# WangWen-Believer/DR-SLAM

Hardware: AMD Instinct MI355X
Metric: RGB-D frames/sec (extract+match) at 640x480 (higher is better)
Workload: dtype u8

## Files before the change

### dr_slam_amd/csrc/drfe_internal.h

```cpp
#ifndef DRFE_INTERNAL_H
#define DRFE_INTERNAL_H

#include <hip/hip_runtime.h>
#ifndef DRFE_NO_ROCTX
#include <roctracer/roctx.h>
#else
static inline int roctxRangePushA(const char*) { return 0; }
static inline int roctxRangePop() { return 0; }
#endif
#include <stdint.h>
#include <time.h>
#include <string>
#include <vector>

#include "../../include/drfe.h"
#include "../../include/drfe_debug.h"

#define DRFE_MAX_LEVELS 16
#define DRFE_EDGE 19
#define DRFE_HALF_PATCH 15
#define DRFE_GRID_COLS 64
#define DRFE_GRID_ROWS 48
#define DRFE_GRID_CELLS (DRFE_GRID_COLS * DRFE_GRID_ROWS)
#define DRFE_FASTC_MAX_EW 38
#define DRFE_FASTC_MAX_RPL 12
#define DRFE_FAST_MAX_WIN 60
#define DRFE_QT_MAX_NODES 1024
#define DRFE_MATCH_MAX_CAND 256

struct DevLevel {
    int w, h;
    int pyrPitch, pyrOff;
    int blurPitch, blurOff;
    int quota;
    int minBX, minBY, maxBX, maxBY;
    int nCols, nRows, wCell, hCell;
    int candCap, candOff;
    int kpCap, kpOff;
    int nIni;
    float hX;
    float scale;
    float kpSize;
    int xtabOff, ytabOff;
    int xwinOff, ywinOff;
    int resizeLds;
    int cellBegin, cellEnd;
    int tileBegin, tileEnd;
};

struct DevGeom {
    int nlevels;
    int iniTh, minTh;
    int imgW, imgH;
    int pyrSlotBytes, blurSlotBytes;
    int candSlotElems, kpSlotElems;
    int totalCells, totalTiles;
    int fastMaxWh;
    int fastCols;
    int fastColsSmall;
    int fastColsRows;
    DevLevel lv[DRFE_MAX_LEVELS];
};

#ifndef DRFE_CC_LINE
#define DRFE_CC_LINE 32
#endif
#define DRFE_CC_SLOT (DRFE_MAX_LEVELS * DRFE_CC_LINE)
#define DRFE_CC_IDX(slot, level) ((size_t)(slot) * DRFE_CC_SLOT + (size_t)(level) * DRFE_CC_LINE)

struct FastCell {
    uint16_t x0, y0;
    uint8_t ww, wh;
    uint8_t level, off;
    uint16_t offX, offY;
    uint32_t cellIdx;
    uint32_t srcOff;
    uint32_t pitch;
    uint32_t candOff, candCap;
    uint8_t ncp, nrb, rpl, pad;
    uint32_t ncpMagic;
};

struct BlurTile { uint16_t tx, ty; uint16_t level, pad; };

struct ResizeTap { uint16_t s0, s1; int16_t w0, w1; };

#include "undistort_math.h"

struct drfe_ctx {
    drfe_config cfg;
    int device;
    hipStream_t stream;
    std::string err;

    std::vector<float> scale, invScale, sigma2, invSigma2;
    std::vector<int> quota;
    int umax[DRFE_HALF_PATCH + 1];
    DevGeom geom;
// ... 128 lines not shown
{
    (void)roctxRangePushA(drfe_stage_name(stage));
    if (c->profile) { (void)hipEventRecord(c->ev[stage][0], s); c->evUsed[stage] = true; }
}
static inline void prof_end(drfe_ctx* c, int stage, hipStream_t s)
{
    if (c->profile) (void)hipEventRecord(c->ev[stage][1], s);
    (void)roctxRangePop();
}
struct DrfeRange {
    explicit DrfeRange(const char* name) { (void)roctxRangePushA(name); }
    ~DrfeRange() { (void)roctxRangePop(); }
};

static inline hipError_t drfe_event_wait_sleeping(hipEvent_t ev)
{
    for (int spins = 0;; spins++) {
        const hipError_t e = hipEventQuery(ev);
        if (e != hipErrorNotReady) return e;
        if (spins < 4) continue;
        struct timespec ts = {0, spins < 40 ? 20000 : 100000};
        nanosleep(&ts, nullptr);
    }
}

void drfe_pool_cpu_add(int pool, long long ns);
struct DrfePoolCpuScope {
    int pool; struct timespec t0;
    explicit DrfePoolCpuScope(int p) : pool(p) { clock_gettime(CLOCK_THREAD_CPUTIME_ID, &t0); }
    ~DrfePoolCpuScope() { struct timespec t1; clock_gettime(CLOCK_THREAD_CPUTIME_ID, &t1); drfe_pool_cpu_add(pool, (t1.tv_sec - t0.tv_sec) * 1000000000LL + (t1.tv_nsec - t0.tv_nsec)); }
};

hipError_t drfe_long_kernel_stream(hipStream_t* s, int part);

int drfe_default_host_threads();
void drfe_cape_lanes_free(drfe_ctx* c);
void drfe_bow_slot_invalidate(drfe_ctx* c, int slot);
void drfe_one_shot_free(drfe_ctx* c);
void drfe_frame_lanes_free(drfe_ctx* c);

int drfe_build_tables(drfe_ctx* c);
int drfe_build_geometry(drfe_ctx* c, int w, int h, DevGeom* g, std::vector<FastCell>* cells,
                        std::vector<BlurTile>* tiles, std::vector<ResizeTap>* taps);

hipError_t drfe_launch_orb(drfe_ctx* c, const uint8_t* d_gray, size_t frameStride, size_t rowStride, int nframes,
                           hipStream_t s);
hipError_t drfe_launch_glue(drfe_ctx* c, const uint16_t* d_depth, size_t frameStride, size_t rowStride,
                            const drfe_camera& cam, int nframes, hipStream_t s);
hipError_t drfe_launch_grid(drfe_ctx* c, const drfe_camera& cam, int nframes, hipStream_t s);
hipError_t drfe_launch_kp_pixels(drfe_ctx* c, int nframes, uint32_t* d_uv, hipStream_t s);
hipError_t drfe_launch_match_consecutive(drfe_ctx* c, const drfe_camera& cam, float th, int mono, int checkOri,
                                         int nframes, hipStream_t s);

#define DRFE_RESIZE_LDS_WD 88
#define DRFE_RESIZE_LDS_ROWS 24
static inline uint32_t drfe_div_magic(uint32_t d) { return d <= 1 ? 0u : (uint32_t)(((1ull << 32) + d - 1) / d); }
#if defined(__HIPCC__)
__device__ __forceinline__ uint32_t drfe_div_by(uint32_t n, uint32_t d, uint32_t magic)
{
    if (!magic) return n;
    uint32_t q = __umulhi(n, magic);
    if (q * d > n) q--;
    return q;
}
__device__ __forceinline__ int drfe_wave_incl_scan(int v, int lane)
{
    v += __builtin_amdgcn_update_dpp(0, v, 0x111, 0xf, 0xf, true);
    v += __builtin_amdgcn_update_dpp(0, v, 0x112, 0xf, 0xf, true);
    v += __builtin_amdgcn_update_dpp(0, v, 0x114, 0xf, 0xf, true);
    v += __builtin_amdgcn_update_dpp(0, v, 0x118, 0xf, 0xf, true);
    const int t0 = __builtin_amdgcn_readlane(v, 15), t1 = __builtin_amdgcn_readlane(v, 31), t2 = __builtin_amdgcn_readlane(v, 47);
    return v + (lane >= 16 ? t0 : 0) + (lane >= 32 ? t1 : 0) + (lane >= 48 ? t2 : 0);
}

__device__ __forceinline__ int drfe_wave_sum_i32(int v)
{
    v += __builtin_amdgcn_update_dpp(0, v, 0xB1, 0xf, 0xf, false);
    v += __builtin_amdgcn_update_dpp(0, v, 0x4E, 0xf, 0xf, false);
    v += __builtin_amdgcn_update_dpp(0, v, 0x124, 0xf, 0xf, false);
    v += __builtin_amdgcn_update_dpp(0, v, 0x128, 0xf, 0xf, false);
    return __builtin_amdgcn_readlane(v, 0) + __builtin_amdgcn_readlane(v, 16) + __builtin_amdgcn_readlane(v, 32) + __builtin_amdgcn_readlane(v, 48);
}
__device__ __forceinline__ uint32_t drfe_wave_min_u32(uint32_t v)
{
    v = min(v, (uint32_t)__builtin_amdgcn_update_dpp(0, (int)v, 0xB1, 0xf, 0xf, false));
    v = min(v, (uint32_t)__builtin_amdgcn_update_dpp(0, (int)v, 0x4E, 0xf, 0xf, false));
    v = min(v, (uint32_t)__builtin_amdgcn_update_dpp(0, (int)v, 0x124, 0xf, 0xf, false));
    v = min(v, (uint32_t)__builtin_amdgcn_update_dpp(0, (int)v, 0x128, 0xf, 0xf, false));
    const uint32_t a = (uint32_t)__builtin_amdgcn_readlane((int)v, 0), b = (uint32_t)__builtin_amdgcn_readlane((int)v, 16),
                   c = (uint32_t)__builtin_amdgcn_readlane((int)v, 32), d = (uint32_t)__builtin_amdgcn_readlane((int)v, 48);
    return min(min(a, b), min(c, d));
}

__device__ __forceinline__ void drfe_xcd_swizzle_2d(uint32_t magic, int& lx, int& ly)
{
    const uint32_t gx = gridDim.x, nwg = gx * gridDim.y;
    const uint32_t orig = blockIdx.y * gx + blockIdx.x;
    const uint32_t q = nwg >> 3, r = nwg & 7, xcd = orig & 7, j = orig >> 3;
    const uint32_t swz = (xcd < r ? xcd * (q + 1) : r * (q + 1) + (xcd - r) * q) + j;
    const uint32_t y = drfe_div_by(swz, gx, magic);
    lx = (int)(swz - y * gx);
    ly = (int)y;
}
__device__ __forceinline__ void drfe_xcd_swizzle_3d(uint32_t magicXY, uint32_t magicX, int& lx, int& ly, int& lz)
{
    const uint32_t gx = gridDim.x, gxy = gx * gridDim.y, nwg = gxy * gridDim.z;
    const uint32_t orig = blockIdx.z * gxy + blockIdx.y * gx + blockIdx.x;
    const uint32_t q = nwg >> 3, r = nwg & 7, xcd = orig & 7, j = orig >> 3;
// ... 29 lines not shown
```

### dr_slam_amd/csrc/orb_geometry.cpp

```cpp
#include "drfe_internal.h"
#include "../../include/drfe_math.h"

#include <algorithm>
#include <cmath>

static inline int align_up(int v, int a) { return (v + a - 1) / a * a; }

int drfe_build_tables(drfe_ctx* c)
{
    const int nl = c->cfg.nlevels;
    const double sfd = (double)c->cfg.scale_factor;
    c->scale.assign(nl, 1.f); c->sigma2.assign(nl, 1.f);
    c->invScale.assign(nl, 1.f); c->invSigma2.assign(nl, 1.f);
    for (int i = 1; i < nl; i++) {
        c->scale[i] = (float)(c->scale[i - 1] * sfd);
        c->sigma2[i] = c->scale[i] * c->scale[i];
    }
    for (int i = 0; i < nl; i++) {
        c->invScale[i] = 1.0f / c->scale[i];
        c->invSigma2[i] = 1.0f / c->sigma2[i];
    }
    c->quota.assign(nl, 0);
    const float factor = (float)(1.0f / sfd);
    float want = c->cfg.nfeatures * (1 - factor) / (1 - (float)std::pow((double)factor, (double)nl));
    int sum = 0;
    for (int l = 0; l < nl - 1; l++) {
        c->quota[l] = drfe_round_half_even(want);
        sum += c->quota[l];
        want *= factor;
    }
    c->quota[nl - 1] = std::max(c->cfg.nfeatures - sum, 0);
    const int hp = DRFE_HALF_PATCH;
    for (int v = 0; v <= hp; v++) c->umax[v] = 0;
    const int vmax = (int)std::floor(hp * std::sqrt(2.f) / 2 + 1);
    const int vmin = (int)std::ceil(hp * std::sqrt(2.f) / 2);
    const double hp2 = hp * hp;
    for (int v = 0; v <= vmax; ++v) c->umax[v] = drfe_round_half_even_d(std::sqrt(hp2 - v * v));
    for (int v = hp, v0 = 0; v >= vmin; --v) {
        while (c->umax[v0] == c->umax[v0 + 1]) ++v0;
        c->umax[v] = v0;
        ++v0;
    }
    return DRFE_OK;
}

static void build_taps_axis(int src, int dst, std::vector<ResizeTap>* out)
{
    const double inv = (double)dst / src;
    const double scale = 1. / inv;
    for (int d = 0; d < dst; d++) {
        float f = (float)((d + 0.5) * scale - 0.5);
        int s = (int)std::floor(f);
        f -= s;
        if (s < 0) { s = 0; f = 0; }
        if (s >= src - 1) { s = src - 1; f = 0; }
        ResizeTap t;
        t.s0 = (uint16_t)s;
        t.s1 = (uint16_t)std::min(s + 1, src - 1);
        int w0 = drfe_round_half_even((1.f - f) * 2048.f), w1 = drfe_round_half_even(f * 2048.f);
        t.w0 = (int16_t)std::min(32767, std::max(-32768, w0));
        t.w1 = (int16_t)std::min(32767, std::max(-32768, w1));
        out->push_back(t);
    }
}

static void build_taps(int src, int dst, int padded, std::vector<ResizeTap>* out)
{
    std::vector<ResizeTap> axis;
    build_taps_axis(src, dst, &axis);
    if (out->size() & 1) out->push_back(ResizeTap{0, 0, 0, 0});
    const int bordered = dst + 2 * DRFE_EDGE;
    for (int b = 0; b < padded; b++) {
        if (b >= bordered) { ResizeTap z = out->back(); z.w0 = z.w1 = 0; out->push_back(z); continue; }
        int p = b - DRFE_EDGE;
        if (p < 0) p = -p;
        if (p >= dst) p = 2 * (dst - 1) - p;
        out->push_back(axis[p]);
    }
}

int drfe_build_geometry(drfe_ctx* c, int w, int h, DevGeom* g, std::vector<FastCell>* cells,
                        std::vector<BlurTile>* tiles, std::vector<ResizeTap>* taps)
{
    const int nl = c->cfg.nlevels;
    g->nlevels = nl;
    g->iniTh = c->cfg.ini_th_fast;
    g->minTh = c->cfg.min_th_fast;
    g->imgW = w; g->imgH = h;
    g->fastMaxWh = 7;
    g->fastCols = 1;
    g->fastColsRows = 7;
    int pyrOff = 0, blurOff = 0, candOff = 0, kpOff = 0;
    if (cells) cells->clear();
    if (tiles) tiles->clear();
    if (taps) taps->clear();
    for (int l = 0; l < nl; l++) {
        DevLevel& L = g->lv[l];
        L.w = drfe_round_half_even((float)w * c->invScale[l]);
        L.h = drfe_round_half_even((float)h * c->invScale[l]);
        L.quota = c->quota[l];
        L.scale = c->scale[l];
        L.kpSize = (float)(int)(31 * c->scale[l]);
        L.minBX = DRFE_EDGE - 3; L.minBY = DRFE_EDGE - 3;
        L.maxBX = L.w - DRFE_EDGE + 3; L.maxBY = L.h - DRFE_EDGE + 3;
        const float width = (float)(L.maxBX - L.minBX), height = (float)(L.maxBY - L.minBY);
        L.nCols = (int)(width / 30.f);
        L.nRows = (int)(height / 30.f);
        if (L.nCols <= 0 || L.nRows <= 0) {
            c->err = "pyramid level " + std::to_string(l) + " is smaller than one 30-px FAST cell";
            return DRFE_ERR_INVALID;
        }
        L.wCell = (int)std::ceil(width / L.nCols);
        L.hCell = (int)std::ceil(height / L.nRows);
        if (L.wCell + 6 > DRFE_FAST_MAX_WIN || L.hCell + 6 > DRFE_FAST_MAX_WIN) {
            c->err = "FAST cell window exceeds the LDS tile";
            return DRFE_ERR_INVALID;
        }
        L.nIni = (int)std::round((float)(L.maxBX - L.minBX) / (L.maxBY - L.minBY));
        if (L.nIni < 1) {
            c->err = "frame aspect ratio gives zero quadtree root nodes (reference divides by zero)";
            return DRFE_ERR_INVALID;
        }
        L.hX = (float)(L.maxBX - L.minBX) / L.nIni;
        L.pyrPitch = align_up(L.w + 2 * DRFE_EDGE, 64);
        L.pyrOff = pyrOff;
        pyrOff += align_up(L.pyrPitch * (L.h + 2 * DRFE_EDGE), 256);
        L.blurPitch = (L.w + DRFE_BTILE_W - 1) / DRFE_BTILE_W;
        L.blurOff = blurOff;
        blurOff += align_up(L.blurPitch * ((L.h + DRFE_BTILE_H - 1) / DRFE_BTILE_H) * 128, 256);
        L.cellBegin = cells ? (int)cells->size() : 0;
// ... 6 lines not shown
            for (int j = 0; j < L.nCols; j++) {
                const float iniX = (float)(L.minBX + j * L.wCell);
                float maxX = iniX + L.wCell + 6;
                if (iniX >= L.maxBX - 6) continue;
                if (maxX > L.maxBX) maxX = (float)L.maxBX;
                FastCell fc;
                fc.x0 = (uint16_t)iniX; fc.y0 = (uint16_t)iniY;
                const int ww = (int)maxX - (int)iniX, wh = (int)maxY - (int)iniY;
                if (ww < 7 || wh < 7) continue;
                fc.ww = (uint8_t)ww; fc.wh = (uint8_t)wh;
                fc.level = (uint8_t)l;
                fc.off = (uint8_t)((fc.x0 + DRFE_EDGE) & 3);
                fc.srcOff = (uint32_t)(L.pyrOff + (fc.y0 + DRFE_EDGE) * L.pyrPitch + (fc.x0 + DRFE_EDGE - fc.off));
                fc.pitch = (uint32_t)L.pyrPitch;
                fc.candOff = 0; fc.candCap = 0;
                fc.offX = (uint16_t)(j * L.wCell); fc.offY = (uint16_t)(i * L.hCell);
                fc.cellIdx = (uint32_t)(i * L.nCols + j);
                {
                    const int ew = ww - 6, eh = wh - 6;
                    const int ncp = (ew + 1) / 2, nrb0 = std::min(64 / ncp, eh);
                    const int rpl = (eh + nrb0 - 1) / nrb0;
                    const int nrb = (eh + rpl - 1) / rpl;
                    fc.ncp = (uint8_t)ncp; fc.nrb = (uint8_t)nrb; fc.rpl = (uint8_t)rpl; fc.pad = 0;
                    fc.ncpMagic = (uint32_t)((65536 + ncp - 1) / ncp);
                    g->fastColsRows = std::max(g->fastColsRows, std::max(nrb * rpl + 6, wh));
                    if (ew > DRFE_FASTC_MAX_EW || rpl > DRFE_FASTC_MAX_RPL) g->fastCols = 0;
                }
                if (cells) cells->push_back(fc);
                if (wh > g->fastMaxWh) g->fastMaxWh = wh;
                candCap += ((ww - 6 + 1) / 2) * ((wh - 6 + 1) / 2);
            }
        }
        L.cellEnd = cells ? (int)cells->size() : 0;
        L.candCap = align_up(std::max(candCap, 64), 64);
        L.candOff = candOff;
        if (cells)
            for (int k = L.cellBegin; k < L.cellEnd; k++) { (*cells)[k].candOff = (uint32_t)L.candOff; (*cells)[k].candCap = (uint32_t)L.candCap; }
        candOff += L.candCap;
        L.kpCap = std::max(L.quota, 4 * L.nIni) + 4;
        if (L.kpCap > DRFE_QT_MAX_NODES) {
            c->err = "nfeatures too large for the quadtree node pool";
            return DRFE_ERR_CAPACITY;
        }
        L.kpOff = kpOff;
        kpOff += L.kpCap;
        L.tileBegin = tiles ? (int)tiles->size() : 0;
        for (int ty = 0; ty < (L.h + DRFE_BLUR_TH - 1) / DRFE_BLUR_TH; ty++)
            for (int tx = 0; tx < (L.w + DRFE_BLUR_TW - 1) / DRFE_BLUR_TW; tx++) {
                BlurTile t; t.tx = (uint16_t)tx; t.ty = (uint16_t)ty; t.level = (uint16_t)l; t.pad = 0;
                if (tiles) tiles->push_back(t);
            }
        L.tileEnd = tiles ? (int)tiles->size() : 0;
        L.xtabOff = L.ytabOff = 0;
        L.xwinOff = L.ywinOff = 0;
        L.resizeLds = 0;
        if (l > 0 && taps) {
            if (taps->size() & 1) taps->push_back(ResizeTap{0, 0, 0, 0});
            L.xtabOff = (int)taps->size();
            build_taps(g->lv[l - 1].w, L.w, L.pyrPitch, taps);
            if (taps->size() & 1) taps->push_back(ResizeTap{0, 0, 0, 0});
            L.ytabOff = (int)taps->size();
            build_taps(g->lv[l - 1].h, L.h, align_up(L.h + 2 * DRFE_EDGE, 4), taps);
            const int bh = L.h + 2 * DRFE_EDGE;
            const int nbx = (L.pyrPitch + 255) / 256, nby = (bh + 15) / 16;
            L.resizeLds = 1;
            L.xwinOff = (int)taps->size();
            for (int b = 0; b < nbx; b++) {
                int lo = 1 << 30, hi = -1;
                for (int x = b * 256; x < std::min(b * 256 + 256, L.pyrPitch); x++) {
                    const ResizeTap& t = (*taps)[L.xtabOff + x];
                    lo = std::min(lo, (int)t.s0); hi = std::max(hi, (int)t.s1);
                }
                const int ws = (lo + DRFE_EDGE) & ~3;
                if ((hi + DRFE_EDGE - ws) / 4 + 1 > DRFE_RESIZE_LDS_WD) L.resizeLds = 0;
                taps->push_back(ResizeTap{(uint16_t)lo, (uint16_t)hi, 0, 0});
            }
            L.ywinOff = (int)taps->size();
            for (int b = 0; b < nby; b++) {
                int lo = 1 << 30, hi = -1;
                for (int y = b * 16; y < std::min(b * 16 + 16, bh); y++) {
                    const ResizeTap& t = (*taps)[L.ytabOff + y];
                    lo = std::min(lo, (int)t.s0); hi = std::max(hi, (int)t.s1);
                }
                if (hi - lo + 1 > DRFE_RESIZE_LDS_ROWS) L.resizeLds = 0;
                taps->push_back(ResizeTap{(uint16_t)lo, (uint16_t)hi, 0, 0});
            }
            if (!L.resizeLds) {
                for (int x = 0; x + 3 < L.pyrPitch; x += 4) {
                    int lo = 1 << 30, hi = -1;
                    for (int k = 0; k < 4; k++) {
                        const ResizeTap& t = (*taps)[L.xtabOff + x + k];
                        lo = std::min(lo, (int)t.s0); hi = std::max(hi, (int)t.s1);
                    }
                    if (hi + DRFE_EDGE - ((lo + DRFE_EDGE) & ~3) > 11) {
                        c->err = "pyramid scale factor too large for the resize kernels (supported: up to 2.0)";
                        return DRFE_ERR_INVALID;
                    }
                }
            }
        }
    }
    g->fastColsSmall = 0;
    if (cells) {
        std::stable_partition(cells->begin(), cells->end(), [](const FastCell& f) { return f.rpl <= 8; });
        for (const FastCell& f : *cells) g->fastColsSmall += f.rpl <= 8 ? 1 : 0;
    }
    g->pyrSlotBytes = pyrOff;
    g->blurSlotBytes = blurOff;
    g->candSlotElems = candOff;
    g->kpSlotElems = kpOff;
    g->totalCells = cells ? (int)cells->size() : 0;
    g->totalTiles = tiles ? (int)tiles->size() : 0;
    return DRFE_OK;
}
```

### dr_slam_amd/csrc/orb_kernels.hip

```cpp
#include "drfe_internal.h"
#include "../../include/drfe_math.h"

#define WAVE 64

__device__ __forceinline__ int reflect101(int p, int n)
{
    if (p < 0) p = -p;
    if (p >= n) p = 2 * (n - 1) - p;
    return p;
}


#define PYR0_ROWS 2
__global__ __launch_bounds__(256) void k_pyr_level0_wide(const DevLevel L, int pyrSlotBytes, const uint8_t* __restrict__ gray,
                                                         size_t frameStride, size_t rowStride, int x16First, int x16Last,
                                                         uint8_t* __restrict__ pyr)
{
    const int slot = blockIdx.z;
    const int y0 = (blockIdx.y * 4 + threadIdx.y) * PYR0_ROWS;
    const int x16 = x16First + (blockIdx.x * 64 + threadIdx.x) * 16;
    const int bh = L.h + 2 * DRFE_EDGE;
    if (y0 >= bh || x16 > x16Last) return;
    const int sx = x16 - DRFE_EDGE;
    const uint8_t* frame = gray + (size_t)slot * frameStride;
// ... 45 lines not shown
#define PYR_ROWS 4
__global__ __launch_bounds__(256) void k_pyr_resize(const DevLevel L, const DevLevel P, int pyrSlotBytes,
                                                    const ResizeTap* __restrict__ taps, uint8_t* __restrict__ pyr)
{
    const int slot = blockIdx.z;
    const int y0 = (blockIdx.y * 4 + threadIdx.y) * PYR_ROWS;
    const int x4 = (blockIdx.x * 64 + threadIdx.x) * 4;
    const int bh = L.h + 2 * DRFE_EDGE;
    if (y0 >= bh || x4 >= L.pyrPitch) return;
    uint8_t* base = pyr + (size_t)slot * pyrSlotBytes;
    const uint4 tya = *reinterpret_cast<const uint4*>(taps + L.ytabOff + y0);
    const uint4 tyb = *reinterpret_cast<const uint4*>(taps + L.ytabOff + y0 + 2);
    const uint4 ta = *reinterpret_cast<const uint4*>(taps + L.xtabOff + x4);
    const uint4 tb = *reinterpret_cast<const uint4*>(taps + L.xtabOff + x4 + 2);
    const uint32_t syp[PYR_ROWS] = {tya.x, tya.z, tyb.x, tyb.z}, wyp[PYR_ROWS] = {tya.y, tya.w, tyb.y, tyb.w};
    const uint32_t sp[4] = {ta.x, ta.z, tb.x, tb.z};
    const uint32_t wp[4] = {ta.y, ta.w, tb.y, tb.w};
    int lo = 0xFFFF;
#pragma unroll
    for (int k = 0; k < 4; k++) lo = min(lo, (int)(sp[k] & 0xFFFF));
    const int ws = (lo + DRFE_EDGE) & ~3;
    const uint8_t* srcw = base + P.pyrOff + (size_t)DRFE_EDGE * P.pyrPitch + ws;
    uint32_t a[PYR_ROWS][3], c[PYR_ROWS][3];
#pragma unroll
    for (int r = 0; r < PYR_ROWS; r++) {
        const uint32_t* R0 = reinterpret_cast<const uint32_t*>(srcw + (size_t)(syp[r] & 0xFFFF) * P.pyrPitch);
        const uint32_t* R1 = reinterpret_cast<const uint32_t*>(srcw + (size_t)(syp[r] >> 16) * P.pyrPitch);
        a[r][0] = R0[0]; a[r][1] = R0[1]; a[r][2] = R0[2];
        c[r][0] = R1[0]; c[r][1] = R1[1]; c[r][2] = R1[2];
    }
    int o0[4], o1[4], w0[4], w1[4];
#pragma unroll
    for (int k = 0; k < 4; k++) {
        o0[k] = (int)(sp[k] & 0xFFFF) + DRFE_EDGE - ws; o1[k] = (int)(sp[k] >> 16) + DRFE_EDGE - ws;
        w0[k] = (int)(short)(wp[k] & 0xFFFF); w1[k] = (int)(short)(wp[k] >> 16);
    }
#pragma unroll
    for (int r = 0; r < PYR_ROWS; r++) {
        if (y0 + r >= bh) break;
        const int b0 = (int)(short)(wyp[r] & 0xFFFF), b1 = (int)(short)(wyp[r] >> 16);
        uint32_t out = 0;
#pragma unroll
        for (int k = 0; k < 4; k++) {
            const int h0 = (int)pick_byte(a[r][0], a[r][1], a[r][2], o0[k]) * w0[k] + (int)pick_byte(a[r][0], a[r][1], a[r][2], o1[k]) * w1[k];
            const int h1 = (int)pick_byte(c[r][0], c[r][1], c[r][2], o0[k]) * w0[k] + (int)pick_byte(c[r][0], c[r][1], c[r][2], o1[k]) * w1[k];
            int v = (((b0 * (h0 >> 4)) >> 16) + ((b1 * (h1 >> 4)) >> 16) + 2) >> 2;
            v = min(255, max(0, v));
            out |= (uint32_t)v << (8 * k);
        }
        *reinterpret_cast<uint32_t*>(base + L.pyrOff + (size_t)(y0 + r) * L.pyrPitch + x4) = out;
    }
}

#define RES_PITCH (DRFE_RESIZE_LDS_WD * 4 + 4)
__global__ __launch_bounds__(256) void k_pyr_resize_lds(const DevLevel L, const DevLevel P, int pyrSlotBytes,
                                                        const ResizeTap* __restrict__ taps, uint8_t* __restrict__ pyr,
                                                        uint32_t magicXY, uint32_t magicX)
{
    __shared__ __attribute__((aligned(16))) uint8_t tile[DRFE_RESIZE_LDS_ROWS * RES_PITCH];
    int bx, by, bz;
    drfe_xcd_swizzle_3d(magicXY, magicX, bx, by, bz);
    bx = __builtin_amdgcn_readfirstlane(bx); by = __builtin_amdgcn_readfirstlane(by);
    const int slot = __builtin_amdgcn_readfirstlane(bz);
    const int tid = threadIdx.y * 64 + threadIdx.x;
    uint8_t* base = pyr + (size_t)slot * pyrSlotBytes;
    const ResizeTap wx = taps[L.xwinOff + bx], wy = taps[L.ywinOff + by];
    const int y0 = (by * 4 + __builtin_amdgcn_readfirstlane((int)threadIdx.y)) * PYR_ROWS;
    const int x4 = (bx * 64 + threadIdx.x) * 4;
    const int bh = L.h + 2 * DRFE_EDGE;
    const bool active = y0 < bh && x4 < L.pyrPitch;
    const int yT = y0 < bh ? y0 : 0, xT = active ? x4 : 0;
    const uint4 tya = *reinterpret_cast<const uint4*>(taps + L.ytabOff + yT);
    const uint4 tyb = *reinterpret_cast<const uint4*>(taps + L.ytabOff + yT + 2);
    const uint4 ta = *reinterpret_cast<const uint4*>(taps + L.xtabOff + xT);
    const uint4 tb = *reinterpret_cast<const uint4*>(taps + L.xtabOff + xT + 2);
    {
        const int r0 = by * (4 * PYR_ROWS);
        if (r0 + 4 * PYR_ROWS <= DRFE_EDGE || r0 >= DRFE_EDGE + L.h) return;
    }
    const int ws = ((int)wx.s0 + DRFE_EDGE) & ~3;
    const int wd = (((int)wx.s1 + DRFE_EDGE - ws) >> 2) + 1;
    const int nr = (int)wy.s1 - (int)wy.s0 + 1;
    const uint8_t* srcw = base + P.pyrOff + (size_t)((int)wy.s0 + DRFE_EDGE) * P.pyrPitch + ws;
    {
        const int q256 = 256 / wd, r256 = 256 - q256 * wd;
        int r = tid / wd, cdw = tid - r * wd;
        while (r < nr) {
            *reinterpret_cast<uint32_t*>(&tile[r * RES_PITCH + cdw * 4]) =
                *reinterpret_cast<const uint32_t*>(srcw + (size_t)r * P.pyrPitch + cdw * 4);
            r += q256; cdw += r256;
            if (cdw >= wd) { cdw -= wd; r++; }
        }
    }
    __syncthreads();
    if (y0 >= bh) return;
    if (y0 + PYR_ROWS <= DRFE_EDGE || y0 >= DRFE_EDGE + L.h) return;
    uint8_t* const dstLevel = base + L.pyrOff;
    const uint32_t syp[PYR_ROWS] = {tya.x, tya.z, tyb.x, tyb.z}, wyp[PYR_ROWS] = {tya.y, tya.w, tyb.y, tyb.w};
    const uint32_t sp[4] = {ta.x, ta.z, tb.x, tb.z}, wp[4] = {ta.y, ta.w, tb.y, tb.w};
    int o0[4], w0[4], w1[4];
#pragma unroll
    for (int k = 0; k < 4; k++) {
        o0[k] = (int)(sp[k] & 0xFFFF) + DRFE_EDGE - ws;
        w0[k] = (int)(short)(wp[k] & 0xFFFF); w1[k] = (int)(short)(wp[k] >> 16);
    }
    auto hrow = [&](int srow, uint32_t (&H)[4]) {
        const uint8_t* R = &tile[srow * RES_PITCH];
#pragma unroll
        for (int k = 0; k < 4; k++) {
            typedef const volatile __attribute__((address_space(3))) uint8_t* lds_u8p;
            lds_u8p q = (lds_u8p)(R + o0[k]);
            H[k] = (uint32_t)(((int)q[0] * w0[k] + (int)q[1] * w1[k]) >> 4);
        }
    };
    int prevB = -1;
    uint32_t Hp[4] = {0, 0, 0, 0};
#pragma unroll
    for (int r = 0; r < PYR_ROWS; r++) {
        if (y0 + r >= bh) break;
        const int pr = y0 + r - DRFE_EDGE;
        if (pr < 0 || pr >= L.h) continue;
        const uint32_t sy = (uint32_t)__builtin_amdgcn_readfirstlane((int)syp[r]), wy2 = (uint32_t)__builtin_amdgcn_readfirstlane((int)wyp[r]);
        const int a = (int)(sy & 0xFFFF) - (int)wy.s0, b = (int)(sy >> 16) - (int)wy.s0;
        uint32_t Ha[4], Hb[4];
        if (a == prevB) {
#pragma unroll
            for (int k = 0; k < 4; k++) Ha[k] = Hp[k];
        } else hrow(a, Ha);
        if (b == a) {
#pragma unroll
            for (int k = 0; k < 4; k++) Hb[k] = Ha[k];
        } else hrow(b, Hb);
        const uint32_t b0s = wy2 << 16, b1s = wy2 & 0xFFFF0000u;
        uint32_t sm[4];
#pragma unroll
        for (int k = 0; k < 4; k++) sm[k] = __umulhi(Ha[k], b0s) + __umulhi(Hb[k], b1s) + 2u;
        typedef unsigned short u16x2r __attribute__((ext_vector_type(2)));
        const u16x2r two = {2, 2};
        const uint32_t q01 = __builtin_bit_cast(uint32_t, __builtin_bit_cast(u16x2r, sm[0] | (sm[1] << 16)) >> two);
        const uint32_t q23 = __builtin_bit_cast(uint32_t, __builtin_bit_cast(u16x2r, sm[2] | (sm[3] << 16)) >> two);
        const uint32_t out = __builtin_amdgcn_perm(q23, q01, 0x06040200u);
        if (active) {
            *reinterpret_cast<uint32_t*>(dstLevel + (uint32_t)(__umul24((uint32_t)(y0 + r), (uint32_t)L.pyrPitch) + (uint32_t)x4)) = out;
            if (pr >= 1 && pr <= DRFE_EDGE)
                *reinterpret_cast<uint32_t*>(dstLevel + (uint32_t)(__umul24((uint32_t)(DRFE_EDGE - pr), (uint32_t)L.pyrPitch) + (uint32_t)x4)) = out;
            if (pr >= L.h - 1 - DRFE_EDGE && pr <= L.h - 2)
                *reinterpret_cast<uint32_t*>(dstLevel + (uint32_t)(__umul24((uint32_t)(DRFE_EDGE + 2 * (L.h - 1) - pr), (uint32_t)L.pyrPitch) + (uint32_t)x4)) = out;
        }
        prevB = b;
#pragma unroll
        for (int k = 0; k < 4; k++) Hp[k] = Hb[k];
    }
}


typedef short s16x2 __attribute__((ext_vector_type(2)));
__device__ __forceinline__ s16x2 pk2(uint32_t lo, uint32_t hi) { return __builtin_bit_cast(s16x2, lo | (hi << 16)); }
__device__ __forceinline__ s16x2 pmin(s16x2 a, s16x2 b) { return __builtin_elementwise_min(a, b); }
__device__ __forceinline__ s16x2 pmax(s16x2 a, s16x2 b) { return __builtin_elementwise_max(a, b); }
typedef unsigned short u16x2 __attribute__((ext_vector_type(2)));
__device__ __forceinline__ u16x2 umax2(u16x2 a, u16x2 b) { return __builtin_elementwise_max(a, b); }
__device__ __forceinline__ u16x2 umin2(u16x2 a, u16x2 b) { return __builtin_elementwise_min(a, b); }

typedef _Float16 h16x2 __attribute__((ext_vector_type(2)));
__device__ __forceinline__ h16x2 hpk(uint32_t lo, uint32_t hi) { return __builtin_bit_cast(h16x2, lo | (hi << 16)); }
__device__ __forceinline__ h16x2 hmin(h16x2 a, h16x2 b) { return __builtin_elementwise_minimum(a, b); }
__device__ __forceinline__ h16x2 hmax(h16x2 a, h16x2 b) { return __builtin_elementwise_maximum(a, b); }
__device__ __forceinline__ h16x2 hmin3(h16x2 a, h16x2 b, h16x2 c) { return hmin(hmin(a, b), c); }
__device__ __forceinline__ h16x2 hmax3(h16x2 a, h16x2 b, h16x2 c) { return hmax(hmax(a, b), c); }

__device__ __forceinline__ h16x2 hpair(const uint8_t* c, int i, int P) { return hpk(c[i], c[i + P]); }
__device__ __forceinline__ uint32_t fast_strength2(const uint8_t* c, const int P)
{
    const int C = 3 * P + 3;
    const h16x2 v = hpair(c, C, P);
    h16x2 d[16];
#define RING(k, o) d[k] = hpair(c, C + (o), P)
    RING(0, 3 * P);       RING(1, 3 * P + 1);   RING(2, 2 * P + 2);    RING(3, P + 3);
    RING(4, 3);           RING(5, -P + 3);      RING(6, -2 * P + 2);   RING(7, -3 * P + 1);
    RING(8, -3 * P);      RING(9, -3 * P - 1);  RING(10, -2 * P - 2);  RING(11, -P - 3);
    RING(12, -3);         RING(13, P - 3);      RING(14, 2 * P - 2);   RING(15, 3 * P - 1);
#undef RING
    h16x2 lo2[8], hi2[8], lo4[8], hi4[8], t[8], u[8];
#pragma unroll
    for (int m = 0; m < 8; m++) {
        lo2[m] = hmin(d[2 * m + 1], d[(2 * m + 2) & 15]);
        hi2[m] = hmax(d[2 * m + 1], d[(2 * m + 2) & 15]);
    }
#pragma unroll
    for (int m = 0; m < 8; m++) { lo4[m] = hmin(lo2[m], lo2[(m + 1) & 7]); hi4[m] = hmax(hi2[m], hi2[(m + 1) & 7]); }
#pragma unroll
    for (int m = 0; m < 8; m++) {
        const h16x2 e0 = d[2 * m], e1 = d[(2 * m + 9) & 15];
        t[m] = hmin3(lo4[m], lo4[(m + 2) & 7], hmax(e0, e1));
        u[m] = hmax3(hi4[m], hi4[(m + 2) & 7], hmin(e0, e1));
    }
    const h16x2 a = hmax(hmax3(hmax3(t[0], t[1], t[2]), t[3], t[4]), hmax3(t[5], t[6], t[7]));
    const h16x2 b = hmin(hmin3(hmin3(u[0], u[1], u[2]), u[3], u[4]), hmin3(u[5], u[6], u[7]));
    const h16x2 one = __builtin_bit_cast(h16x2, 0x00010001u), zero = __builtin_bit_cast(h16x2, 0u);
    const h16x2 r = hmax(hmax(a - v, v - b) - one, zero);
    return __builtin_bit_cast(uint32_t, r);
// ... 956 lines not shown
            reinterpret_cast<ulonglong2*>(drow)[0] = make_ulonglong2(w4[0], w4[1]);
            reinterpret_cast<ulonglong2*>(drow)[1] = make_ulonglong2(w4[2], w4[3]);
            const DevLevel& L = G->lv[level[j]];
            drfe_keypoint kp;
            kp.x = (float)xi[j]; kp.y = (float)yi[j];
            if (level[j] != 0) { kp.x *= L.scale; kp.y *= L.scale; }
            kp.size = L.kpSize;
            kp.angle = angle[j];
            kp.response = (float)resp[j];
            kp.octave = level[j];
            kp.class_id = -1;
            kps[(size_t)slot * maxKp + g] = kp;
        }
    }
}



__global__ void k_clear_counts(int* __restrict__ candCount, int n, int* __restrict__ status)
{
    const int i = blockIdx.x * 256 + threadIdx.x;
    if (i < n) candCount[(size_t)i * DRFE_CC_LINE] = 0;
    if (i == 0) status[0] = 0;
}

hipError_t drfe_launch_orb(drfe_ctx* c, const uint8_t* d_gray, size_t frameStride, size_t rowStride, int nframes,
                           hipStream_t s)
{
    const DevGeom& g = c->geom;
    const int nl = g.nlevels;
    hipError_t e;
    hipLaunchKernelGGL(k_clear_counts, dim3((nframes * DRFE_CC_SLOT / DRFE_CC_LINE + 255) / 256), dim3(256), 0, s, c->d_candCount, nframes * DRFE_CC_SLOT / DRFE_CC_LINE, c->d_status);
    e = hipGetLastError();
    if (e != hipSuccess) return e;

    prof_begin(c, DRFE_STAGE_PYRAMID, s);
    {
        const DevLevel& L = g.lv[0];
        const int bh = L.h + 2 * DRFE_EDGE;
        const bool aligned16 = (((uintptr_t)d_gray | frameStride | rowStride) & 15) == 0;
        int x16First = 32, x16Last = (L.w / 16) * 16, leftEnd = 0, rightBegin = 0;
        if (aligned16 && x16Last >= x16First) {
            const int nWide = (x16Last - x16First) / 16 + 1;
            hipLaunchKernelGGL(k_pyr_level0_wide, dim3((nWide + 63) / 64, (bh + 4 * PYR0_ROWS - 1) / (4 * PYR0_ROWS), nframes),
                               dim3(64, 4), 0, s, L, g.pyrSlotBytes, d_gray, frameStride, rowStride, x16First, x16Last, c->d_pyr);
            leftEnd = x16First; rightBegin = x16Last + 16;
        }
        const int nEdge = leftEnd / 4 + (L.pyrPitch - rightBegin) / 4;
        hipLaunchKernelGGL(k_pyr_level0_edge, dim3((nEdge * bh + 255) / 256, nframes), dim3(256), 0, s, L,
                           g.pyrSlotBytes, d_gray, frameStride, rowStride, leftEnd, rightBegin, c->d_pyr);
    }
    for (int l = 1; l < nl; l++) {
        const DevLevel& L = g.lv[l];
        dim3 grid((L.pyrPitch / 4 + 63) / 64, (L.h + 2 * DRFE_EDGE + 4 * PYR_ROWS - 1) / (4 * PYR_ROWS), nframes);
        if (L.resizeLds)
            hipLaunchKernelGGL(k_pyr_resize_lds, grid, dim3(64, 4), 0, s, L, g.lv[l - 1], g.pyrSlotBytes, c->d_taps, c->d_pyr,
                               drfe_div_magic(grid.x * grid.y), drfe_div_magic(grid.x));
        else
            hipLaunchKernelGGL(k_pyr_resize, grid, dim3(64, 4), 0, s, L, g.lv[l - 1], g.pyrSlotBytes, c->d_taps, c->d_pyr);
    }
    prof_end(c, DRFE_STAGE_PYRAMID, s);

    prof_begin(c, DRFE_STAGE_FAST, s);
    if (g.fastCols && !c->fastGeneric) {
        const int nSmall = g.fastColsSmall, nBig = g.totalCells - nSmall;
        if (nSmall > 0)
            hipLaunchKernelGGL((k_fast_cells_cols<8>), dim3(nSmall, nframes), dim3(64), (size_t)fastc_lds_bytes(g.fastColsRows, 8 * 64), s,
                               c->d_cells, g.nlevels, g.pyrSlotBytes, g.candSlotElems, g.iniTh, g.minTh, c->d_pyr, c->d_cand0,
                               c->d_cand1, c->d_candCount, c->d_status, drfe_div_magic((uint32_t)nSmall), 0, c->fastScreen, fastc_list_off(g.fastColsRows), fastc_list_cap(g.fastColsRows, 8 * 64));
        if (nBig > 0) {
            prof_end(c, DRFE_STAGE_FAST, s);
            prof_begin(c, DRFE_STAGE_FAST_B, s);
        }
        if (nBig > 0)
            hipLaunchKernelGGL((k_fast_cells_cols<DRFE_FASTC_MAX_RPL>), dim3(nBig, nframes), dim3(64),
                               (size_t)fastc_lds_bytes(g.fastColsRows, DRFE_FASTC_MAX_RPL * 64), s, c->d_cells, g.nlevels, g.pyrSlotBytes, g.candSlotElems,
                               g.iniTh, g.minTh, c->d_pyr, c->d_cand0, c->d_cand1, c->d_candCount, c->d_status,
                               drfe_div_magic((uint32_t)nBig), nSmall, c->fastScreen, fastc_list_off(g.fastColsRows), fastc_list_cap(g.fastColsRows, DRFE_FASTC_MAX_RPL * 64));
        if (nBig > 0) prof_end(c, DRFE_STAGE_FAST_B, s);
        else prof_end(c, DRFE_STAGE_FAST, s);
    } else {
        hipLaunchKernelGGL(k_fast_cells, dim3(g.totalCells, nframes), dim3(64), (size_t)fast_lds_bytes(g.fastMaxWh), s, c->d_cells,
                           g.nlevels, g.pyrSlotBytes, g.candSlotElems, g.iniTh, g.minTh, c->d_pyr,
                           c->d_cand0, c->d_cand1, c->d_candCount, c->d_status, fast_sc_off(g.fastMaxWh),
                           drfe_div_magic((uint32_t)g.totalCells));
        prof_end(c, DRFE_STAGE_FAST, s);
    }

    prof_begin(c, DRFE_STAGE_QUADTREE, s);
    {
        int nBig = 0, capMax = 0;
        for (int l = 0; l < nl; l++) {
            if (g.lv[l].w * g.lv[l].h > 160000 || g.lv[l].kpCap > 256) nBig = l + 1;
            capMax = std::max(capMax, g.lv[l].kpCap);
        }
        if (nl * nframes <= 2 * 256) nBig = nl;
        if (nBig > 0) {
            if (capMax > 256)
                hipLaunchKernelGGL((k_quadtree<512, 16, DRFE_QT_MAX_NODES>), dim3(nBig, nframes), dim3(512), 0, s, c->d_geom, 0,
                                   c->d_cand0, c->d_cand1, c->d_node, c->d_candCount, c->d_sel, c->d_selCount, c->d_status);
            else
                hipLaunchKernelGGL((k_quadtree<512, 16, 256>), dim3(nBig, nframes), dim3(512), 0, s, c->d_geom, 0, c->d_cand0,
                                   c->d_cand1, c->d_node, c->d_candCount, c->d_sel, c->d_selCount, c->d_status);
        }
        if (nBig < nl)
            hipLaunchKernelGGL((k_quadtree<256, 8, 256>), dim3(nl - nBig, nframes), dim3(256), 0, s, c->d_geom, nBig, c->d_cand0,
                               c->d_cand1, c->d_node, c->d_candCount, c->d_sel, c->d_selCount, c->d_status);
    }
    prof_end(c, DRFE_STAGE_QUADTREE, s);

    prof_begin(c, DRFE_STAGE_BLUR, s);
    hipLaunchKernelGGL(k_blur, dim3(g.totalTiles, nframes), dim3(256), 0, s, c->d_geom, c->d_tiles, c->d_pyr,
// ... 13 lines not shown
```

Before: 268,900.

## Replace 2D LDS pyramid resize with 1D packed-tile kernel using per-block windows

Rewrites the pyramid resize LDS kernel as a 1D grid of 256-thread blocks over only the rows actually needed. Each block's source window is precomputed on the host and loaded with 16-byte vector loads into a dynamically sized LDS tile, with the load count set by a FILL template parameter. Horizontal taps now use byte permute plus udot2 instead of per-byte LDS reads. Idle blocks over border-only rows are dropped and the row grouping is tuned to reduce wasted threads, at the cost of more complex host planning and several template instantiations.

```diff
diff --git a/dr_slam_amd/csrc/drfe_internal.h b/dr_slam_amd/csrc/drfe_internal.h
--- a/dr_slam_amd/csrc/drfe_internal.h
+++ b/dr_slam_amd/csrc/drfe_internal.h
@@ -42,8 +42,10 @@
     float scale;
     float kpSize;
     int xtabOff, ytabOff;
-    int xwinOff, ywinOff;
     int resizeLds;
+    int rzRow0, rzGroups, rzCols, rzBlocks;
+    int rzRows, rzWq, rzFill, rzWinOff;
+    uint32_t rzColsMagic, rzWqMagic;
     int cellBegin, cellEnd;
     int tileBegin, tileEnd;
 };
@@ -278,8 +280,9 @@
 hipError_t drfe_launch_match_consecutive(drfe_ctx* c, const drfe_camera& cam, float th, int mono, int checkOri,
                                          int nframes, hipStream_t s);
 
-#define DRFE_RESIZE_LDS_WD 88
-#define DRFE_RESIZE_LDS_ROWS 24
+#define DRFE_RESIZE_BLOCK 256
+#define DRFE_RESIZE_MAX_FILL 8
+#define DRFE_RESIZE_TILE_BYTES 32768
 static inline uint32_t drfe_div_magic(uint32_t d) { return d <= 1 ? 0u : (uint32_t)(((1ull << 32) + d - 1) / d); }
 #if defined(__HIPCC__)
 __device__ __forceinline__ uint32_t drfe_div_by(uint32_t n, uint32_t d, uint32_t magic)
diff --git a/dr_slam_amd/csrc/orb_geometry.cpp b/dr_slam_amd/csrc/orb_geometry.cpp
--- a/dr_slam_amd/csrc/orb_geometry.cpp
+++ b/dr_slam_amd/csrc/orb_geometry.cpp
@@ -3,6 +3,7 @@
 
 #include <algorithm>
 #include <cmath>
+#include <cstdlib>
 
 static inline int align_up(int v, int a) { return (v + a - 1) / a * a; }
 
@@ -76,6 +77,57 @@
         if (p < 0) p = -p;
         if (p >= dst) p = 2 * (dst - 1) - p;
         out->push_back(axis[p]);
+    }
+}
+
+static void plan_resize_tile(DevLevel& L, const DevLevel& P, std::vector<ResizeTap>* taps)
+{
+    const int bw = L.w + 2 * DRFE_EDGE, bh = L.h + 2 * DRFE_EDGE, B = DRFE_RESIZE_BLOCK;
+    const int cols = (bw + 3) / 4;
+    int groups = 0, blocks = 0;
+    for (int ng = (L.h + 3) / 4; 4 * ng <= bh; ng++) {
+        const int nb = (ng * cols + B - 1) / B;
+        if (!groups || (long long)ng * cols * blocks > (long long)groups * cols * nb) { groups = ng; blocks = nb; }
+    }
+    const int extra = 4 * groups - L.h;
+    L.rzCols = cols; L.rzGroups = groups; L.rzBlocks = blocks;
+    L.rzRow0 = DRFE_EDGE - std::max(0, extra - DRFE_EDGE);
+    L.rzColsMagic = drfe_div_magic((uint32_t)cols);
+    bool ok = true;
+    const ResizeTap* xt = taps->data() + L.xtabOff;
+    const ResizeTap* yt = taps->data() + L.ytabOff;
+    for (int x = 0; x < 4 * cols; x += 2)
+        if (std::abs((int)xt[x].s0 - (int)xt[x + 1].s0) > 2) ok = false;
+    std::vector<int> r0v(blocks), c0v(blocks);
+    int rows = 0, quads = 0;
+    for (int b = 0; b < blocks; b++) {
+        const int i0 = b * B, i1 = std::min(groups * cols, i0 + B);
+        int r0 = 1 << 30, r1 = -1, c0 = 1 << 30, c1 = -1;
+        for (int g = i0 / cols; g <= (i1 - 1) / cols; g++) {
+            for (int y = L.rzRow0 + 4 * g; y < L.rzRow0 + 4 * g + 4; y++) {
+                r0 = std::min(r0, (int)yt[y].s0 + DRFE_EDGE); r1 = std::max(r1, (int)yt[y].s1 + DRFE_EDGE);
+            }
+            const int ca = std::max(i0 - g * cols, 0), cb = std::min(i1 - g * cols, cols);
+            for (int x = 4 * ca; x < 4 * cb; x++) {
+                c0 = std::min(c0, (int)xt[x].s0 + DRFE_EDGE); c1 = std::max(c1, (int)xt[x].s0 + 1 + DRFE_EDGE);
+            }
+        }
+        r0v[b] = r0; c0v[b] = c0 & ~15;
+        rows = std::max(rows, r1 - r0 + 1);
+        quads = std::max(quads, (c1 - c0v[b]) / 16 + 1);
+    }
+    const int pbh = P.h + 2 * DRFE_EDGE;
+    if (rows > pbh || 16 * quads > P.pyrPitch) ok = false;
+    quads = std::max(quads, 2);
+    L.rzRows = rows; L.rzWq = quads;
+    L.rzWqMagic = drfe_div_magic((uint32_t)quads);
+    L.rzFill = (rows * quads + B - 1) / B;
+    if (L.rzFill > DRFE_RESIZE_MAX_FILL || rows * quads * 16 + 16 > DRFE_RESIZE_TILE_BYTES) ok = false;
+    L.resizeLds = ok ? 1 : 0;
+    L.rzWinOff = (int)taps->size();
+    for (int b = 0; b < blocks; b++) {
+        const int r0 = std::max(0, std::min(r0v[b], pbh - rows)), c0 = std::max(0, std::min(c0v[b], P.pyrPitch - 16 * quads));
+        taps->push_back(ResizeTap{(uint16_t)r0, (uint16_t)c0, 0, 0});
     }
 }
 
@@ -188,8 +240,9 @@
             }
         L.tileEnd = tiles ? (int)tiles->size() : 0;
         L.xtabOff = L.ytabOff = 0;
-        L.xwinOff = L.ywinOff = 0;
         L.resizeLds = 0;
+        L.rzRow0 = L.rzGroups = L.rzCols = L.rzBlocks = L.rzRows = L.rzWq = L.rzFill = L.rzWinOff = 0;
+        L.rzColsMagic = L.rzWqMagic = 0;
         if (l > 0 && taps) {
             if (taps->size() & 1) taps->push_back(ResizeTap{0, 0, 0, 0});
             L.xtabOff = (int)taps->size();
@@ -197,31 +250,8 @@
             if (taps->size() & 1) taps->push_back(ResizeTap{0, 0, 0, 0});
             L.ytabOff = (int)taps->size();
             build_taps(g->lv[l - 1].h, L.h, align_up(L.h + 2 * DRFE_EDGE, 4), taps);
-            const int bh = L.h + 2 * DRFE_EDGE;
-            const int nbx = (L.pyrPitch + 255) / 256, nby = (bh + 15) / 16;
-            L.resizeLds = 1;
-            L.xwinOff = (int)taps->size();
-            for (int b = 0; b < nbx; b++) {
-                int lo = 1 << 30, hi = -1;
-                for (int x = b * 256; x < std::min(b * 256 + 256, L.pyrPitch); x++) {
-                    const ResizeTap& t = (*taps)[L.xtabOff + x];
-                    lo = std::min(lo, (int)t.s0); hi = std::max(hi, (int)t.s1);
-                }
-                const int ws = (lo + DRFE_EDGE) & ~3;
-                if ((hi + DRFE_EDGE - ws) / 4 + 1 > DRFE_RESIZE_LDS_WD) L.resizeLds = 0;
-                taps->push_back(ResizeTap{(uint16_t)lo, (uint16_t)hi, 0, 0});
-            }
-            L.ywinOff = (int)taps->size();
-            for (int b = 0; b < nby; b++) {
-                int lo = 1 << 30, hi = -1;
-                for (int y = b * 16; y < std::min(b * 16 + 16, bh); y++) {
-                    const ResizeTap& t = (*taps)[L.ytabOff + y];
-                    lo = std::min(lo, (int)t.s0); hi = std::max(hi, (int)t.s1);
-                }
-                if (hi - lo + 1 > DRFE_RESIZE_LDS_ROWS) L.resizeLds = 0;
-                taps->push_back(ResizeTap{(uint16_t)lo, (uint16_t)hi, 0, 0});
-            }
-            if (!L.resizeLds) {
+            plan_resize_tile(L, g->lv[l - 1], taps);
+            {
                 for (int x = 0; x + 3 < L.pyrPitch; x += 4) {
                     int lo = 1 << 30, hi = -1;
                     for (int k = 0; k < 4; k++) {
diff --git a/dr_slam_amd/csrc/orb_kernels.hip b/dr_slam_amd/csrc/orb_kernels.hip
--- a/dr_slam_amd/csrc/orb_kernels.hip
+++ b/dr_slam_amd/csrc/orb_kernels.hip
@@ -121,76 +121,81 @@
     }
 }
 
-#define RES_PITCH (DRFE_RESIZE_LDS_WD * 4 + 4)
-__global__ __launch_bounds__(256) void k_pyr_resize_lds(const DevLevel L, const DevLevel P, int pyrSlotBytes,
-                                                        const ResizeTap* __restrict__ taps, uint8_t* __restrict__ pyr,
-                                                        uint32_t magicXY, uint32_t magicX)
-{
-    __shared__ __attribute__((aligned(16))) uint8_t tile[DRFE_RESIZE_LDS_ROWS * RES_PITCH];
-    int bx, by, bz;
-    drfe_xcd_swizzle_3d(magicXY, magicX, bx, by, bz);
-    bx = __builtin_amdgcn_readfirstlane(bx); by = __builtin_amdgcn_readfirstlane(by);
-    const int slot = __builtin_amdgcn_readfirstlane(bz);
-    const int tid = threadIdx.y * 64 + threadIdx.x;
-    uint8_t* base = pyr + (size_t)slot * pyrSlotBytes;
-    const ResizeTap wx = taps[L.xwinOff + bx], wy = taps[L.ywinOff + by];
-    const int y0 = (by * 4 + __builtin_amdgcn_readfirstlane((int)threadIdx.y)) * PYR_ROWS;
-    const int x4 = (bx * 64 + threadIdx.x) * 4;
-    const int bh = L.h + 2 * DRFE_EDGE;
-    const bool active = y0 < bh && x4 < L.pyrPitch;
-    const int yT = y0 < bh ? y0 : 0, xT = active ? x4 : 0;
-    const uint4 tya = *reinterpret_cast<const uint4*>(taps + L.ytabOff + yT);
-    const uint4 tyb = *reinterpret_cast<const uint4*>(taps + L.ytabOff + yT + 2);
-    const uint4 ta = *reinterpret_cast<const uint4*>(taps + L.xtabOff + xT);
-    const uint4 tb = *reinterpret_cast<const uint4*>(taps + L.xtabOff + xT + 2);
+template <int FILL>
+__global__ __launch_bounds__(256) void k_pyr_resize_tile(const DevLevel L, const DevLevel P, int pyrSlotBytes,
+                                                         const ResizeTap* __restrict__ taps, uint8_t* __restrict__ pyr,
+                                                         uint32_t magicBlocks)
+{
+    extern __shared__ __attribute__((aligned(16))) uint8_t tile[];
+    int bx, slot;
+    drfe_xcd_swizzle_2d(magicBlocks, bx, slot);
+    bx = __builtin_amdgcn_readfirstlane(bx); slot = __builtin_amdgcn_readfirstlane(slot);
+    const int tid = threadIdx.x;
+    uint8_t* const base = pyr + (size_t)slot * pyrSlotBytes;
+    const uint32_t winp = ((const __attribute__((address_space(4))) uint32_t*)taps)[2 * (L.rzWinOff + bx)];
+    const struct { uint32_t s0, s1; } win = {winp & 0xFFFFu, winp >> 16};
+    const uint32_t nItems = (uint32_t)(L.rzGroups * L.rzCols);
+    uint32_t item = (uint32_t)(bx * DRFE_RESIZE_BLOCK + tid);
+    const bool active = item < nItems;
+    if (!active) item = nItems - 1;
+    auto divm = [](uint32_t n, uint32_t d, uint32_t magic) { const uint32_t q = __umulhi(n, magic); return q * d > n ? q - 1 : q; };
+    const uint32_t g = divm(item, (uint32_t)L.rzCols, L.rzColsMagic);
+    const int y0 = L.rzRow0 + 4 * (int)g, x4 = 4 * (int)(item - g * (uint32_t)L.rzCols);
+    const uint8_t* const tb8 = reinterpret_cast<const uint8_t*>(taps);
+    const uint32_t tyo = (uint32_t)(L.ytabOff + y0) * 8u, txo = (uint32_t)(L.xtabOff + x4) * 8u;
+    const uint2 t0 = *reinterpret_cast<const uint2*>(tb8 + tyo), t1 = *reinterpret_cast<const uint2*>(tb8 + (tyo + 8u));
+    const uint2 t2 = *reinterpret_cast<const uint2*>(tb8 + (tyo + 16u)), t3 = *reinterpret_cast<const uint2*>(tb8 + (tyo + 24u));
+    const uint4 ta = *reinterpret_cast<const uint4*>(tb8 + txo);
+    const uint4 tb = *reinterpret_cast<const uint4*>(tb8 + (txo + 16u));
     {
-        const int r0 = by * (4 * PYR_ROWS);
-        if (r0 + 4 * PYR_ROWS <= DRFE_EDGE || r0 >= DRFE_EDGE + L.h) return;
-    }
-    const int ws = ((int)wx.s0 + DRFE_EDGE) & ~3;
-    const int wd = (((int)wx.s1 + DRFE_EDGE - ws) >> 2) + 1;
-    const int nr = (int)wy.s1 - (int)wy.s0 + 1;
-    const uint8_t* srcw = base + P.pyrOff + (size_t)((int)wy.s0 + DRFE_EDGE) * P.pyrPitch + ws;
-    {
-        const int q256 = 256 / wd, r256 = 256 - q256 * wd;
-        int r = tid / wd, cdw = tid - r * wd;
-        while (r < nr) {
-            *reinterpret_cast<uint32_t*>(&tile[r * RES_PITCH + cdw * 4]) =
-                *reinterpret_cast<const uint32_t*>(srcw + (size_t)r * P.pyrPitch + cdw * 4);
-            r += q256; cdw += r256;
-            if (cdw >= wd) { cdw -= wd; r++; }
-        }
+        const uint8_t* const srcw = base + P.pyrOff + (uint32_t)((int)win.s0 * P.pyrPitch + (int)win.s1);
+        const uint32_t nq = (uint32_t)(L.rzRows * L.rzWq), tpitch = (uint32_t)L.rzWq * 16u;
+        uint4 v[FILL];
+        uint32_t dst[FILL];
+#pragma unroll
+        for (int k = 0; k < FILL; k++) {
+            const uint32_t j = (uint32_t)tid + (uint32_t)(k * DRFE_RESIZE_BLOCK), jc = j < nq ? j : 0u;
+            const uint32_t r = divm(jc, (uint32_t)L.rzWq, L.rzWqMagic), q = jc - r * (uint32_t)L.rzWq;
+            v[k] = *reinterpret_cast<const uint4*>(srcw + (__umul24(r, (uint32_t)P.pyrPitch) + q * 16u));
+            dst[k] = j < nq ? __umul24(r, tpitch) + q * 16u : nq * 16u;
+        }
+#pragma unroll
+        for (int k = 0; k < FILL; k++) *reinterpret_cast<uint4*>(&tile[dst[k]]) = v[k];
     }
     __syncthreads();
-    if (y0 >= bh) return;
-    if (y0 + PYR_ROWS <= DRFE_EDGE || y0 >= DRFE_EDGE + L.h) return;
+    if (!active) return;
+    const uint32_t tpitch = (uint32_t)L.rzWq * 16u;
+    const uint32_t sp[4] = {ta.x, ta.z, tb.x, tb.z}, wp[4] = {ta.y, ta.w, tb.y, tb.w};
+    int o[4];
+#pragma unroll
+    for (int k = 0; k < 4; k++) o[k] = (int)(sp[k] & 0xFFFFu) + DRFE_EDGE - (int)win.s1;
+    const uint32_t p01 = (uint32_t)min(o[0], o[1]) & ~3u, p23 = (uint32_t)min(o[2], o[3]) & ~3u;
+    uint32_t sel[4];
+#pragma unroll
+    for (int k = 0; k < 4; k++) {
+        const uint32_t rel = (uint32_t)o[k] - (k < 2 ? p01 : p23);
+        sel[k] = rel | ((rel + 1u) << 16) | 0x0C000C00u;
+    }
+    typedef unsigned short u16x2v __attribute__((ext_vector_type(2)));
+    auto hrow = [&](int srow, uint32_t (&H)[4]) {
+        const uint32_t* A = reinterpret_cast<const uint32_t*>(&tile[(uint32_t)srow * tpitch + p01]);
+        const uint32_t* C = reinterpret_cast<const uint32_t*>(&tile[(uint32_t)srow * tpitch + p23]);
+        const uint32_t a0 = A[0], a1 = A[1], c0 = C[0], c1 = C[1];
+        const uint32_t pr[4] = {__builtin_amdgcn_perm(a1, a0, sel[0]), __builtin_amdgcn_perm(a1, a0, sel[1]),
+                                __builtin_amdgcn_perm(c1, c0, sel[2]), __builtin_amdgcn_perm(c1, c0, sel[3])};
+#pragma unroll
+        for (int k = 0; k < 4; k++)
+            H[k] = __builtin_amdgcn_udot2(__builtin_bit_cast(u16x2v, pr[k]), __builtin_bit_cast(u16x2v, wp[k]), 0u, false) >> 4;
+    };
     uint8_t* const dstLevel = base + L.pyrOff;
-    const uint32_t syp[PYR_ROWS] = {tya.x, tya.z, tyb.x, tyb.z}, wyp[PYR_ROWS] = {tya.y, tya.w, tyb.y, tyb.w};
-    const uint32_t sp[4] = {ta.x, ta.z, tb.x, tb.z}, wp[4] = {ta.y, ta.w, tb.y, tb.w};
-    int o0[4], w0[4], w1[4];
-#pragma unroll
-    for (int k = 0; k < 4; k++) {
-        o0[k] = (int)(sp[k] & 0xFFFF) + DRFE_EDGE - ws;
-        w0[k] = (int)(short)(wp[k] & 0xFFFF); w1[k] = (int)(short)(wp[k] >> 16);
-    }
-    auto hrow = [&](int srow, uint32_t (&H)[4]) {
-        const uint8_t* R = &tile[srow * RES_PITCH];
-#pragma unroll
-        for (int k = 0; k < 4; k++) {
-            typedef const volatile __attribute__((address_space(3))) uint8_t* lds_u8p;
-            lds_u8p q = (lds_u8p)(R + o0[k]);
-            H[k] = (uint32_t)(((int)q[0] * w0[k] + (int)q[1] * w1[k]) >> 4);
-        }
-    };
+    const uint2 typ[4] = {t0, t1, t2, t3};
+    const int rowEnd = L.rzRow0 + 4 * L.rzGroups;
     int prevB = -1;
     uint32_t Hp[4] = {0, 0, 0, 0};
 #pragma unroll
-    for (int r = 0; r < PYR_ROWS; r++) {
-        if (y0 + r >= bh) break;
-        const int pr = y0 + r - DRFE_EDGE;
-        if (pr < 0 || pr >= L.h) continue;
-        const uint32_t sy = (uint32_t)__builtin_amdgcn_readfirstlane((int)syp[r]), wy2 = (uint32_t)__builtin_amdgcn_readfirstlane((int)wyp[r]);
-        const int a = (int)(sy & 0xFFFF) - (int)wy.s0, b = (int)(sy >> 16) - (int)wy.s0;
+    for (int r = 0; r < 4; r++) {
+        const uint32_t sy = typ[r].x, wy2 = typ[r].y;
+        const int a = (int)(sy & 0xFFFFu) + DRFE_EDGE - (int)win.s0, b = (int)(sy >> 16) + DRFE_EDGE - (int)win.s0;
         uint32_t Ha[4], Hb[4];
         if (a == prevB) {
 #pragma unroll
@@ -204,18 +209,17 @@
         uint32_t sm[4];
 #pragma unroll
         for (int k = 0; k < 4; k++) sm[k] = __umulhi(Ha[k], b0s) + __umulhi(Hb[k], b1s) + 2u;
-        typedef unsigned short u16x2r __attribute__((ext_vector_type(2)));
-        const u16x2r two = {2, 2};
-        const uint32_t q01 = __builtin_bit_cast(uint32_t, __builtin_bit_cast(u16x2r, sm[0] | (sm[1] << 16)) >> two);
-        const uint32_t q23 = __builtin_bit_cast(uint32_t, __builtin_bit_cast(u16x2r, sm[2] | (sm[3] << 16)) >> two);
+        const u16x2v two = {2, 2};
+        const uint32_t q01 = __builtin_bit_cast(uint32_t, __builtin_bit_cast(u16x2v, sm[0] | (sm[1] << 16)) >> two);
+        const uint32_t q23 = __builtin_bit_cast(uint32_t, __builtin_bit_cast(u16x2v, sm[2] | (sm[3] << 16)) >> two);
         const uint32_t out = __builtin_amdgcn_perm(q23, q01, 0x06040200u);
-        if (active) {
-            *reinterpret_cast<uint32_t*>(dstLevel + (uint32_t)(__umul24((uint32_t)(y0 + r), (uint32_t)L.pyrPitch) + (uint32_t)x4)) = out;
-            if (pr >= 1 && pr <= DRFE_EDGE)
-                *reinterpret_cast<uint32_t*>(dstLevel + (uint32_t)(__umul24((uint32_t)(DRFE_EDGE - pr), (uint32_t)L.pyrPitch) + (uint32_t)x4)) = out;
-            if (pr >= L.h - 1 - DRFE_EDGE && pr <= L.h - 2)
-                *reinterpret_cast<uint32_t*>(dstLevel + (uint32_t)(__umul24((uint32_t)(DRFE_EDGE + 2 * (L.h - 1) - pr), (uint32_t)L.pyrPitch) + (uint32_t)x4)) = out;
-        }
+        const int y = y0 + r, p = y - DRFE_EDGE;
+        *reinterpret_cast<uint32_t*>(dstLevel + (uint32_t)(__umul24((uint32_t)y, (uint32_t)L.pyrPitch) + (uint32_t)x4)) = out;
+        if (p >= 1 && p <= DRFE_EDGE && DRFE_EDGE - p < L.rzRow0)
+            *reinterpret_cast<uint32_t*>(dstLevel + (uint32_t)(__umul24((uint32_t)(DRFE_EDGE - p), (uint32_t)L.pyrPitch) + (uint32_t)x4)) = out;
+        const int yb = DRFE_EDGE + 2 * (L.h - 1) - p;
+        if (p >= L.h - 1 - DRFE_EDGE && p <= L.h - 2 && yb >= rowEnd)
+            *reinterpret_cast<uint32_t*>(dstLevel + (uint32_t)(__umul24((uint32_t)yb, (uint32_t)L.pyrPitch) + (uint32_t)x4)) = out;
         prevB = b;
 #pragma unroll
         for (int k = 0; k < 4; k++) Hp[k] = Hb[k];
@@ -1278,12 +1282,17 @@
     }
     for (int l = 1; l < nl; l++) {
         const DevLevel& L = g.lv[l];
-        dim3 grid((L.pyrPitch / 4 + 63) / 64, (L.h + 2 * DRFE_EDGE + 4 * PYR_ROWS - 1) / (4 * PYR_ROWS), nframes);
-        if (L.resizeLds)
-            hipLaunchKernelGGL(k_pyr_resize_lds, grid, dim3(64, 4), 0, s, L, g.lv[l - 1], g.pyrSlotBytes, c->d_taps, c->d_pyr,
-                               drfe_div_magic(grid.x * grid.y), drfe_div_magic(grid.x));
-        else
+        if (L.resizeLds) {
+            typedef void (*ResizeTileFn)(const DevLevel, const DevLevel, int, const ResizeTap*, uint8_t*, uint32_t);
+            static const ResizeTileFn fns[DRFE_RESIZE_MAX_FILL] = {k_pyr_resize_tile<1>, k_pyr_resize_tile<2>, k_pyr_resize_tile<3>,
+                k_pyr_resize_tile<4>, k_pyr_resize_tile<5>, k_pyr_resize_tile<6>, k_pyr_resize_tile<7>, k_pyr_resize_tile<8>};
+            const dim3 grid(L.rzBlocks, nframes);
+            hipLaunchKernelGGL(fns[L.rzFill - 1], grid, dim3(DRFE_RESIZE_BLOCK), (size_t)(L.rzRows * L.rzWq * 16 + 16), s, L,
+                               g.lv[l - 1], g.pyrSlotBytes, c->d_taps, c->d_pyr, drfe_div_magic(grid.x));
+        } else {
+            const dim3 grid((L.pyrPitch / 4 + 63) / 64, (L.h + 2 * DRFE_EDGE + 4 * PYR_ROWS - 1) / (4 * PYR_ROWS), nframes);
             hipLaunchKernelGGL(k_pyr_resize, grid, dim3(64, 4), 0, s, L, g.lv[l - 1], g.pyrSlotBytes, c->d_taps, c->d_pyr);
+        }
     }
     prof_end(c, DRFE_STAGE_PYRAMID, s);
 
```

Measured after the change: 280,200 (median of 6 runs). +4.2%, better.
